# jzlianglu/pykaldi2

Hardware: AMD Instinct MI355X
Metric: iRTF (hrs audio/hr) 3x512 BLSTM LF-MMI, LibriSpeech-shaped synthetic utterances (higher is better)
Workload: dtype f32 (GEMMs: bf16x3 split, f32 accumulate)

## Files before the change

include/pk2hip.h:

```cpp
#ifndef PK2HIP_H_
#define PK2HIP_H_

#include <stddef.h>
#include <stdint.h>

#ifdef __cplusplus
extern "C" {
#endif

typedef enum {
  PK2_OK = 0,
  PK2_ERR_INVALID = -1,
  PK2_ERR_HIP = -2,
  PK2_ERR_LIMIT = -3,
  PK2_ERR_IO = -4,
  PK2_ERR_NUMERIC = -5
} pk2_status;

const char* pk2_last_error(void);
int pk2_version(void);

typedef struct pk2_den_graph pk2_den_graph;

int pk2_den_graph_create(int32_t num_states, int32_t num_pdfs, int64_t num_arcs,
// ... 212 lines not shown
                                int64_t ignore_index, int64_t rows, int32_t num_classes,
                                float* loss_sum, int32_t* count, float* grad, int64_t grad_row_stride, void* stream);
int pk2_scale_inplace_ratio(float* data, int64_t n, const float* num_dev, const float* den_dev, void* stream);
int pk2_scale_by_count(float* data, int64_t n, float numerator, const int32_t* count_den,
                       void* stream);
int pk2_scale_by_scalars(const float* in, float* out, int64_t n, const float* mul_dev, const int32_t* count_den_dev,
                         void* stream);

int pk2_gemm_f32(int32_t transa, int32_t transb, int32_t M, int32_t N, int32_t K, float alpha,
                 const float* A, int64_t lda, const float* B, int64_t ldb, float beta, float* C,
                 int64_t ldc, const float* bias, void* stream);
int pk2_gemm_f32_act(int32_t transa, int32_t transb, int32_t M, int32_t N, int32_t K, float alpha,
                     const float* A, int64_t lda, const float* B, int64_t ldb, float beta, float* C,
                     int64_t ldc, const float* bias, int32_t act, const float* gate, int64_t ldg, void* stream);
int pk2_gemm_f32_seg(int32_t transa, int32_t transb, int32_t M, int32_t N, int32_t K, int32_t nseg, float alpha,
                     const float* A, int64_t lda, int64_t segA, const float* B, int64_t ldb, int64_t segB, float beta,
                     float* C, int64_t ldc, const float* bias, int32_t act, const float* gate, int64_t ldg,
                     void* stream);
int pk2_gemm_f32_batched(int32_t transa, int32_t transb, int32_t M, int32_t N, int32_t K, float alpha,
                         const float* A, int64_t lda, int64_t strideA0, int64_t strideA1, const float* B,
                         int64_t ldb, int64_t strideB0, int64_t strideB1, float beta, float* C, int64_t ldc,
                         int64_t strideC0, int64_t strideC1, int32_t n0, int32_t n1, void* stream);
int pk2_gemm_set_arith(int32_t arith);
int pk2_gemm_get_arith(void);
int pk2_gemm_f32_tn_colsum(int32_t M, int32_t N, int32_t K, float alpha, const float* A, int64_t lda, const float* B,
                           int64_t ldb, float beta, float* C, int64_t ldc, float* colsum, void* stream);
int pk2_colsum_f32(const float* A, int64_t lda, int32_t M, int32_t N, float beta, float* out,
                   void* stream);

size_t pk2_lstm_fwd_workspace_floats(int32_t B, int32_t H, int32_t num_dirs);
int pk2_lstm_layer_fwd(const float* gx, const float* whh, const float* bhh, int32_t B, int32_t T,
                       int32_t H, int32_t num_dirs, float* y, float* gates, float* cells,
                       void* workspace, void* stream);
int pk2_lstm_persist_status(uint32_t* abort_flag);
#define PK2_LSTM_PATH_NONE 0
#define PK2_LSTM_PATH_SEQ 1
#define PK2_LSTM_PATH_BIG 2
#define PK2_LSTM_PATH_BIG_AG 3
#define PK2_LSTM_PATH_STEP_SMALL 4
#define PK2_LSTM_PATH_STEP_BIG 5
int pk2_lstm_last_path(int32_t* fwd, int32_t* bwd);
size_t pk2_lstm_bwd_scratch_floats(int32_t B, int32_t H, int32_t num_dirs);
int pk2_lstm_layer_bwd(const float* dy, const float* whh, const float* gates, const float* cells,
                       int32_t B, int32_t T, int32_t H, int32_t num_dirs, float* dgx,
                       float* scratch, void* stream);
int pk2_lstm_layer_bwd_bias(const float* dy, const float* whh, const float* gates, const float* cells,
                            int32_t B, int32_t T, int32_t H, int32_t num_dirs, float* dgx, float* scratch,
                            float* dbias_ih, float* dbias_hh, int32_t* bias_done, void* stream);
size_t pk2_lstm_bwd_wgrad_workspace_floats(int32_t B, int32_t H, int32_t num_dirs);
int pk2_lstm_layer_bwd_wgrad(const float* dy, const float* whh, const float* gates, const float* cells, const float* y,
                             int32_t B, int32_t T, int32_t H, int32_t num_dirs, float* dgx, float* scratch,
                             float* dbias_ih, float* dbias_hh, float* dwhh, float* wgrad_ws, int32_t* bias_done,
                             int32_t* whh_done, void* stream);

int pk2_layernorm_fwd(const float* x, const float* res, const float* gamma, const float* beta, int64_t rows,
                      int32_t C, float eps, float* sum_out, float* y, float* mean, float* rstd, void* stream);
int pk2_layernorm_bwd(const float* dy, const float* s, const float* mean, const float* rstd,
                      const float* gamma, int64_t rows, int32_t C, float* ds, float* dgamma, float* dbeta,
                      void* stream);
int pk2_softmax_mask_fwd(float* scores, const float* src_mask, const uint8_t* key_padding, int32_t B, int32_t H,
                         int32_t T, void* stream);
int pk2_softmax_bwd(const float* P, float* dP, int32_t BH, int32_t T, void* stream);

int pk2_attention_fwd(const float* qkv, int32_t T, int32_t B, int32_t H, int32_t head_dim, float scale,
                      const float* src_mask, const uint8_t* key_padding, float dropout_p, uint64_t seed, float* ctx,
                      float* lse, void* stream);
// ... 138 lines not shown
```

pykaldi2_amd/_lib.py:

```python
import ctypes as C
import os

import torch

_HERE = os.path.dirname(os.path.abspath(__file__))
LIB_PATH = os.environ.get("PK2_LIB") or os.path.join(_HERE, "libpk2hip.so")


class Pk2Error(RuntimeError):
    pass


class NumBatch(C.Structure):
    _fields_ = [("arc_src", C.c_void_p), ("arc_dst", C.c_void_p), ("arc_pdf", C.c_void_p),
                ("arc_weight", C.c_void_p), ("frame_off", C.c_void_p), ("state_off", C.c_void_p),
                ("final_state", C.c_void_p), ("final_weight", C.c_void_p), ("final_off", C.c_void_p),
                ("total_arcs", C.c_int64), ("max_seq_arcs", C.c_int64)]


class DecoderOpts(C.Structure):
    _fields_ = [("beam", C.c_float), ("lattice_beam", C.c_float), ("beam_delta", C.c_float),
                ("acoustic_scale", C.c_float), ("max_active", C.c_int32), ("min_active", C.c_int32),
                ("tokens_per_frame", C.c_int32), ("links_per_frame", C.c_int32)]

# ... 137 lines not shown
    "pk2_pad_roll_subsample": (C.c_int, [_vp, _vp, _i32, _i32, _i32, _i32, _vp, _i32, _i32, _vp]),
    "pk2_mvn_apply": (C.c_int, [_vp, _vp, _vp, _i64, _i32, _vp, _vp]),
    "pk2_softmax_ce_fwd_bwd": (C.c_int, [_vp, _i64, _vp, _i64, _i64, _i32, _vp, _vp, _vp, _i64, _vp, _vp]),
    "pk2_softmax_ce_fwd_bwd_mean": (C.c_int, [_vp, _i64, _vp, _i64, _i64, _i32, _vp, _vp, _vp, _i64, _vp]),
    "pk2_scale_inplace_ratio": (C.c_int, [_vp, _i64, _vp, _vp, _vp]),
    "pk2_scale_by_count": (C.c_int, [_vp, _i64, _f32, _vp, _vp]),
    "pk2_scale_by_scalars": (C.c_int, [_vp, _vp, _i64, _vp, _vp, _vp]),
    "pk2_gemm_f32": (C.c_int, [_i32, _i32, _i32, _i32, _i32, _f32, _vp, _i64, _vp, _i64, _f32, _vp, _i64,
                               _vp, _vp]),
    "pk2_gemm_f32_act": (C.c_int, [_i32, _i32, _i32, _i32, _i32, _f32, _vp, _i64, _vp, _i64, _f32, _vp, _i64, _vp, _i32, _vp, _i64,
                                   _vp]),
    "pk2_gemm_f32_seg": (C.c_int, [_i32, _i32, _i32, _i32, _i32, _i32, _f32, _vp, _i64, _i64, _vp, _i64, _i64, _f32, _vp, _i64, _vp,
                                   _i32, _vp, _i64, _vp]),
    "pk2_gemm_f32_batched": (C.c_int, [_i32, _i32, _i32, _i32, _i32, _f32, _vp, _i64, _i64, _i64, _vp, _i64, _i64, _i64,
                                       _f32, _vp, _i64, _i64, _i64, _i32, _i32, _vp]),
    "pk2_gemm_f32_tn_colsum": (C.c_int, [_i32, _i32, _i32, _f32, _vp, _i64, _vp, _i64, _f32, _vp, _i64, _vp, _vp]),
    "pk2_gemm_set_arith": (C.c_int, [_i32]),
    "pk2_gemm_get_arith": (C.c_int, []),
    "pk2_layernorm_fwd": (C.c_int, [_vp, _vp, _vp, _vp, _i64, _i32, _f32, _vp, _vp, _vp, _vp, _vp]),
    "pk2_layernorm_bwd": (C.c_int, [_vp, _vp, _vp, _vp, _vp, _i64, _i32, _vp, _vp, _vp, _vp]),
    "pk2_softmax_mask_fwd": (C.c_int, [_vp, _vp, _vp, _i32, _i32, _i32, _vp]),
    "pk2_softmax_bwd": (C.c_int, [_vp, _vp, _i32, _i32, _vp]),
    "pk2_attention_fwd": (C.c_int, [_vp, _i32, _i32, _i32, _i32, _f32, _vp, _vp, _f32, C.c_uint64, _vp, _vp, _vp]),
    "pk2_attention_bwd": (C.c_int, [_vp, _vp, _vp, _vp, _i32, _i32, _i32, _i32, _f32, _vp, _vp, _f32, C.c_uint64, _vp,
                                    _vp, _vp]),
    "pk2_attention_bwd_part": (C.c_int, [_i32, _vp, _vp, _vp, _vp, _i32, _i32, _i32, _i32, _f32, _vp, _vp, _f32, C.c_uint64,
                                         _vp, _vp, _vp]),
    "pk2_relu_fwd": (C.c_int, [_vp, _i64, _vp]),
    "pk2_relu_bwd": (C.c_int, [_vp, _vp, _i64, _vp]),
    "pk2_add_inplace": (C.c_int, [_vp, _vp, _i64, _vp]),
    "pk2_colsum_f32": (C.c_int, [_vp, _i64, _i32, _i32, _f32, _vp, _vp]),
    "pk2_lstm_fwd_workspace_floats": (_sz, [_i32, _i32, _i32]),
    "pk2_lstm_layer_fwd": (C.c_int, [_vp, _vp, _vp, _i32, _i32, _i32, _i32, _vp, _vp, _vp, _vp, _vp]),
    "pk2_lstm_persist_status": (C.c_int, [C.POINTER(C.c_uint32)]),
    "pk2_lstm_last_path": (C.c_int, [C.POINTER(_i32), C.POINTER(_i32)]),
    "pk2_lattice_determinize": (C.c_int, [_i32, _i32, _i64, _vp, _vp, _vp, _vp, _vp, _vp, _vp, C.c_double, _i64, C.POINTER(_vp)]),
    "pk2_det_lattice_sizes": (C.c_int, [_vp, C.POINTER(_i32), C.POINTER(_i32), C.POINTER(_i64), C.POINTER(_i64), C.POINTER(_i64)]),
    "pk2_det_lattice_export": (C.c_int, [_vp] * 12),
    "pk2_det_lattice_destroy": (None, [_vp]),
    "pk2_persist_guard_status": (C.c_int, [C.POINTER(C.c_uint32)]),
    "pk2_persist_guard_clear": (C.c_int, []),
    "pk2_persist_guard_raise": (C.c_int, [_vp]),
    "pk2_persist_guard_export": (C.c_int, [_vp, _vp]),
    "pk2_persist_guard_import": (C.c_int, [_vp, C.c_uint32, _vp]),
    "pk2_persist_guard_verdict": (C.c_int, [C.c_uint32, C.POINTER(C.c_uint32), C.POINTER(C.c_uint32)]),
    "pk2_lstm_bwd_scratch_floats": (_sz, [_i32, _i32, _i32]),
    "pk2_lstm_layer_bwd_bias": (C.c_int, [_vp, _vp, _vp, _vp, _i32, _i32, _i32, _i32, _vp, _vp, _vp, _vp, C.POINTER(_i32), _vp]),
    "pk2_lstm_layer_bwd": (C.c_int, [_vp, _vp, _vp, _vp, _i32, _i32, _i32, _i32, _vp, _vp, _vp]),
    "pk2_lstm_bwd_wgrad_workspace_floats": (_sz, [_i32, _i32, _i32]),
    "pk2_lstm_layer_bwd_wgrad": (C.c_int, [_vp, _vp, _vp, _vp, _vp, _i32, _i32, _i32, _i32, _vp, _vp, _vp, _vp, _vp, _vp,
                                           C.POINTER(_i32), C.POINTER(_i32), _vp]),
    "pk2_dropout_f32": (C.c_int, [_vp, _vp, _i64, _f32, C.c_uint64, _vp]),
    "pk2_grad_norm": (C.c_int, [_vp, _i64, _vp, _vp, _sz, _vp]),
    "pk2_grad_norm_workspace_bytes": (_sz, [_i64]),
    "pk2_adam_step": (C.c_int, [_vp, _vp, _vp, _vp, _vp, _i64, _f32, _f32, _f32, _f32, _f32, _i64, _f32,
                                _vp, _f32, _vp]),
    "pk2_sgd_step": (C.c_int, [_vp, _vp, _vp, _i64, _f32, _f32, _f32, _i32, _f32, _vp, _f32, _vp]),
    "pk2_stream_create_cu_mask": (C.c_int, [_i32, C.POINTER(_vp)]),
    "pk2_stream_destroy": (C.c_int, [_vp]),
    "pk2_debug_where": (C.c_int, [_vp, _i32, _vp]),
    "pk2_debug_peer_reduce": (C.c_int, [_vp, _vp, _i64, _i32, _i32, _vp]),
}

_lib = None


# ... 61 lines not shown
```

pykaldi2_amd/csrc/lstm.hip:

```cpp
#include <algorithm>

#include "common.h"
#include "gemm_tile.h"
#include "lstm_persist.h"
#include "step_graph.h"

namespace pk2 {

typedef float f32x4 __attribute__((ext_vector_type(4)));

constexpr int kFwdThreads = 256;
constexpr int kFwdUnits = 4;

__device__ __forceinline__ float fast_sigmoid(float x) {
  return __builtin_amdgcn_rcpf(1.0f + __builtin_amdgcn_exp2f(-1.4426950408889634f * x));
}
__device__ __forceinline__ float fast_tanh(float x) {
  return 1.0f - 2.0f * __builtin_amdgcn_rcpf(1.0f + __builtin_amdgcn_exp2f(2.8853900817779268f * x));
}

struct LstmFwdParams {
  const float* gx;
  const float* whh;
  const float* bhh;
// ... 434 lines not shown
    const LstmFwdParams* pbb = slot->params;
    const StepCounter* cb = slot->counter;
    char keyb[64];
    snprintf(keyb, sizeof(keyb), "lstm_fwd_big_H%d_D%d_Z%d_%p", H, D, (int)gridb.z, (void*)stream);
    rc = g_graphs.run(keyb, T, slot->counter, stream, [&](hipStream_t s, int j) {
      hipLaunchKernelGGL(lstm_fwd_step_big, gridb, dim3(256), 0, s, pbb, cb, j);
    });
    if (rc) return rc;
    PK2_LAUNCH_CHECK();
    g_last_fwd_path = PK2_LSTM_PATH_STEP_BIG;
    return PK2_OK;
  }
  const int zf = ((B + 15) / 16 + kFwdTileGroup - 1) / kFwdTileGroup;
  dim3 grid(H / kFwdUnits, D, zf), block(kFwdThreads);
  const LstmFwdParams* pb = slot->params;
  const StepCounter* c = slot->counter;
  char key[64];
  snprintf(key, sizeof(key), "lstm_fwd_H%d_D%d_Z%d_%p", H, D, zf, (void*)stream);
  rc = g_graphs.run(key, T, slot->counter, stream, [&](hipStream_t s, int j) {
    switch (H) {
      case 64: launch_step(lstm_fwd_step<4>, grid, block, s, pb, c, j); break;
      case 128: launch_step(lstm_fwd_step<8>, grid, block, s, pb, c, j); break;
      case 256: launch_step(lstm_fwd_step<16>, grid, block, s, pb, c, j); break;
      case 512: launch_step(lstm_fwd_step<32>, grid, block, s, pb, c, j); break;
      default: launch_step(lstm_fwd_step<64>, grid, block, s, pb, c, j); break;
    }
  });
  if (rc) return rc;
#ifdef PK2_LSTM_PROFILE
  hipLaunchKernelGGL(lstm_prof_print, dim3(1), dim3(1), 0, stream, T - 1);
#endif
  PK2_LAUNCH_CHECK();
  g_last_fwd_path = PK2_LSTM_PATH_STEP_SMALL;
  return PK2_OK;
}

extern "C" int pk2_lstm_persist_status(uint32_t* abort_flag) {
  PK2_REQUIRE(abort_flag, "lstm_persist_status: null pointer");
  PK2_HIP(hipDeviceSynchronize());
  unsigned f = 0, f2 = 0;
  int rc = lstm_seq_status(&f);
  if (!rc) rc = lstm_big_status(&f2);
  *abort_flag = f | f2;
  return rc;
}

extern "C" size_t pk2_lstm_bwd_scratch_floats(int32_t B, int32_t H, int32_t D) {
  return (size_t)D * H * 4 * H + (size_t)D * B * H + 64 + (B >= kBigBatch ? (size_t)kBigSplitK * D * B * H : 0);
}

static int lstm_layer_bwd_impl(const float* dy, const float* whh, const float* gates, const float* cells, int32_t B, int32_t T,
                               int32_t H, int32_t D, float* dgx, float* scratch, float* dbias_ih, float* dbias_hh,
                               int32_t* bias_done, void* stream_, SeqWgradCall* wgrad = nullptr);

extern "C" int pk2_lstm_layer_bwd(const float* dy, const float* whh, const float* gates, const float* cells,
                                  int32_t B, int32_t T, int32_t H, int32_t D, float* dgx, float* scratch,
                                  void* stream_) {
  return lstm_layer_bwd_impl(dy, whh, gates, cells, B, T, H, D, dgx, scratch, nullptr, nullptr, nullptr, stream_);
}

extern "C" int pk2_lstm_layer_bwd_bias(const float* dy, const float* whh, const float* gates, const float* cells,
                                       int32_t B, int32_t T, int32_t H, int32_t D, float* dgx, float* scratch,
                                       float* dbias_ih, float* dbias_hh, int32_t* bias_done, void* stream_) {
  PK2_REQUIRE(bias_done, "lstm_bwd_bias: null bias_done");
  return lstm_layer_bwd_impl(dy, whh, gates, cells, B, T, H, D, dgx, scratch, dbias_ih, dbias_hh, bias_done, stream_);
}
// ... 84 lines not shown
```

pykaldi2_amd/csrc/lstm_persist.h:

```cpp
#pragma once
#include "common.h"

namespace pk2 {

bool lstm_seq_wanted(int B, int H, int D);
int lstm_fwd_seq_launch(const float* gx, const float* whh, const float* bhh, int B, int T, int H, int D, float* y,
                        float* gates, float* cells, hipStream_t stream, bool* ran);
struct SeqWgradCall { const float* y; float* dwhh; float* ws; bool done; };
size_t lstm_seq_wgrad_workspace_floats(int B, int H, int D);
int lstm_bwd_seq_launch(const float* dy, const float* whh, const float* gates, const float* cells, int B, int T, int H,
                        int D, float* dgx, hipStream_t stream, bool* ran, float* dbias_ih = nullptr, float* dbias_hh = nullptr,
                        bool* bias_done = nullptr, SeqWgradCall* wgrad = nullptr);
int lstm_seq_status(unsigned* abort_flag);

bool lstm_big_wanted(int B, int H, int D);
int lstm_fwd_big_launch(const float* gx, const float* whh, const float* bhh, int B, int T, int H, int D, float* y,
                        float* gates, float* cells, hipStream_t stream, bool* ran);
int lstm_bwd_big_launch(const float* dy, const float* whh, const float* gates, const float* cells, int B, int T, int H,
                        int D, float* dgx, hipStream_t stream, bool* ran, bool* all_gather);
int lstm_big_status(unsigned* abort_flag);

}
```

pykaldi2_amd/csrc/lstm_persist_seq.hip:

```cpp
#include <algorithm>
#include <cstdint>
#include <cstdlib>
#include <map>

#include "common.h"
#include "lstm_persist.h"
#include "persist_guard.h"

namespace pk2 {

typedef float f32x4 __attribute__((ext_vector_type(4)));
typedef unsigned u32x4 __attribute__((ext_vector_type(4)));

constexpr unsigned kSeqSentinel = 0x7fc0dead;
constexpr int kSH = 512;
constexpr int kSWgs = 32;
constexpr int kSeqTeams = 8;
constexpr int kSeqMaxTasks = 64;
constexpr long long kSeqSpinTicks = 1000LL * 1000 * 100;
constexpr int kSeqMailDepth = 8;
constexpr int kSeqMailFloats = kSeqMailDepth * kSWgs * kSWgs * 16;

struct SeqCtl {
  unsigned arrive[8];
// ... 282 lines not shown
#ifdef PK2_SEQ_PROFILE
      asm volatile("" : "+v"(s0), "+v"(s1), "+v"(s2), "+v"(s3));
#endif
      SQ_T(2);
      const float x = pre + (l16 == 0 ? s0 : l16 == 1 ? s1 : l16 == 2 ? s2 : s3);
      const float act = fmaf(act_a, __builtin_amdgcn_rcpf(1.0f + __builtin_amdgcn_exp2f(act_s * x)), act_b);
      const float fg = seq_dpp<0x101>(act), gg = seq_dpp<0x102>(act), og = seq_dpp<0x103>(act);
      cstate = fg * cstate + act * gg;
      const float h = og * seq_tanh(cstate);
      if (unit_lane) seq_store(y_out, h);
      y_out += y_stride;
      SQ_T(3);
      if (gate_lane) outs[buf][out_idx] = act;
      if (unit_lane) outs[buf][64 + uw] = cstate;
      if (w == 2) {
        gxs[(step + 2) % 3][lane] = gnext;
        gnext = *gx_in;
        gx_in += step + 4 < T ? gx_stride : 0;
      }
      if (w == 3 && step > 0) {
        *gates_out = outs[buf ^ 1][lane];
        if (lane < 16) *cells_out = outs[buf ^ 1][64 + lane];
        gates_out += gates_stride; cells_out += cells_stride;
      }
      SQ_T(4);
    }
    __syncthreads();
    if (w == 3) {
      *gates_out = outs[(T - 1) & 1][lane];
      if (lane < 16) *cells_out = outs[(T - 1) & 1][64 + lane];
    }
    SQ_PRINT("lstm_fwd_seq2", "(poll | lds + barrier | product + row sums | gates + h store | lds hand-over, wave 2 / 3 traffic)", T);
    if (tid == 0 && rank == 0) __hip_atomic_fetch_add(&ctl->done, 1u, __ATOMIC_RELAXED, __HIP_MEMORY_SCOPE_AGENT);
    if (!seq_team_barrier(ctl, role, &nbar, s_i)) return;
  }
}

typedef float f32x32 __attribute__((ext_vector_type(32)));
struct SeqNoWgrad {};
__device__ __forceinline__ float (*seq_yring())[kSH] {
  __shared__ __attribute__((aligned(16))) float ring[3][kSH];
  return ring;
}
template <bool WGRAD, typename WG>
__device__ __forceinline__ void lstm_bwd_seq2_body(const SeqBwdParams& p, SeqCtl* ctl, const WG& g) {
  constexpr int H = kSH, G4 = 4 * kSH;
  __shared__ __attribute__((aligned(16))) float dgl[64];
  __shared__ __attribute__((aligned(16))) float cst[3][16][8];
  float (*yring)[kSH] = nullptr;
  if constexpr (WGRAD) yring = seq_yring();
  __shared__ int s_i[8];
  const int tid = threadIdx.x, lane = tid & 63, w = tid >> 6;
  SeqRole role;
  if (!seq_register(ctl, s_i, &role)) return;
  const int rank = role.rank, B = p.B, T = p.T, D = p.D;
  float* mail0 = p.mail + (size_t)role.team_index * kSeqMailFloats;
  const u32x4 sent = {kSeqSentinel, kSeqSentinel, kSeqSentinel, kSeqSentinel};
  const int row = lane >> 4, l16 = lane & 15;
  const bool pw_lane = w == 0 && l16 < 4;
  const int pw_unit = (4 * row + l16) & 15;
  const bool io = w == 1;
  const bool io16 = io && lane < 16;
  unsigned nbar = 0;
  for (int iter = 0; iter <= kSeqMaxTasks; ++iter) {
    const int task = seq_next_task(ctl, role, iter, B * D, s_i);
    if (task < 0) return;
// ... 208 lines not shown
  if (threadIdx.x == 0) { *sticky = 1u; persist_guard_raise(guard_dev, guard_host); }
  for (size_t i = threadIdx.x; i < n; i += blockDim.x) out[i] = __uint_as_float(0x7fc00000u);
}

struct SeqExit { unsigned pairs; int fold; float* out; size_t n; unsigned* sticky; unsigned* guard_dev; unsigned* guard_host; float* mail; size_t mail_n; };
__device__ __forceinline__ void seq_exit_check(SeqCtl* ctl, const SeqExit& x) {
  if (!x.fold) return;
  __shared__ unsigned s_last;
  __syncthreads();
  if (threadIdx.x == 0) s_last = __hip_atomic_fetch_add(&ctl->exited, 1u, __ATOMIC_ACQ_REL, __HIP_MEMORY_SCOPE_AGENT) == gridDim.x - 1u ? 1u : 0u;
  __syncthreads();
  if (!s_last) return;
  const bool good = seq_load_u(&ctl->abort) == 0u && seq_load_u(&ctl->done) == x.pairs && x.fold != 2;
  __syncthreads();
  for (unsigned i = threadIdx.x; i < sizeof(SeqCtl) / sizeof(unsigned); i += blockDim.x) reinterpret_cast<unsigned*>(ctl)[i] = 0u;
  if (good) return;
  if (threadIdx.x == 0) { if (x.fold != 2) *x.sticky = 1u; persist_guard_raise(x.guard_dev, x.guard_host); }
  for (size_t i = threadIdx.x; i < x.n; i += blockDim.x) x.out[i] = __uint_as_float(0x7fc00000u);
  for (size_t i = threadIdx.x; i < x.mail_n; i += blockDim.x) x.mail[i] = __uint_as_float(kSeqSentinel);
}
__global__ void __launch_bounds__(256) lstm_fwd_seq2(SeqFwdParams p, SeqCtl* ctl, SeqExit x) {
  lstm_fwd_seq2_body(p, ctl);
  seq_exit_check(ctl, x);
}
__global__ void __launch_bounds__(256) lstm_bwd_seq2(SeqBwdParams p, SeqCtl* ctl, SeqExit x) {
  lstm_bwd_seq2_body<false>(p, ctl, SeqNoWgrad());
  seq_exit_check(ctl, x);
}
__global__ void __launch_bounds__(256) lstm_bwd_seq2_wgrad(SeqBwdParams p, SeqCtl* ctl, SeqExit x, SeqWgradParams g) {
  lstm_bwd_seq2_body<true>(p, ctl, g);
  seq_exit_check(ctl, x);
}

__global__ void __launch_bounds__(256) lstm_seq_wgrad_reduce(const float* __restrict__ ws, float* __restrict__ dwhh, int B, int D,
                                                             const unsigned* __restrict__ sticky) {
  constexpr size_t kSlice = (size_t)4 * kSH * kSH;
  const size_t i = (size_t)blockIdx.x * 256 + threadIdx.x;
  if (*sticky != 0u) {
    dwhh[i] = __uint_as_float(0x7fc00000u);
    return;
  }
  const float* in = ws + i;
  float sum = in[0];
  for (int b = 1; b < B; ++b) sum += in[(size_t)b * D * kSlice];
  dwhh[i] += sum;
}

struct SeqScratch { SeqCtl* ctl = nullptr; float* mail = nullptr; unsigned* sticky = nullptr; PersistGuard guard;
                    int mail_clean_teams = 0;
                    bool ctl_clean = false; };
static std::map<DevStream, SeqScratch> g_seq_scratch;
static PersistFamily g_seq("lstm_seq");

static void seq_mail_dirty() { for (auto& kv : g_seq_scratch) { kv.second.mail_clean_teams = 0; kv.second.ctl_clean = false; } }

static int seq_scratch(hipStream_t stream, SeqScratch** out) {
  static const bool hooked = (persist_guard_on_clear(seq_mail_dirty), true);
  (void)hooked;
  SeqScratch& sc = g_seq_scratch[dev_stream(stream)];
  if (!sc.ctl) PK2_HIP(hipMalloc(reinterpret_cast<void**>(&sc.ctl), sizeof(SeqCtl)));
  if (!sc.mail) PK2_HIP(hipMalloc(reinterpret_cast<void**>(&sc.mail), (size_t)8 * kSeqTeams * kSeqMailFloats * sizeof(float)));
  if (!sc.sticky) { int rc = g_seq.new_sticky(stream, &sc.sticky); if (rc) return rc; }
  if (!sc.guard.dev) { int rc = persist_guard(&sc.guard); if (rc) return rc; }
  *out = &sc;
  return PK2_OK;
}

static int seq_teams(int pairs) { return std::max(1, std::min(2, (pairs + 7) / 8)); }

bool lstm_seq_wanted(int B, int H, int D) {
  const char* env = getenv("PK2_LSTM_SEQ");
  if (env && atoi(env) == 0) return false;
  if (!g_seq.usable() || H != kSH || B < 1 || B * D > 32 || (D != 1 && D != 2)) return false;
  return device_cu_count() == 8 * kSWgs;
}

int lstm_fwd_seq_launch(const float* gx, const float* whh, const float* bhh, int B, int T, int H, int D, float* y,
                        float* gates, float* cells, hipStream_t stream, bool* ran) {
  *ran = false;
  SeqScratch* sc = nullptr;
  int rc = seq_scratch(stream, &sc);
  if (rc) return rc;
  if (!sc->ctl_clean) PK2_HIP(hipMemsetAsync(sc->ctl, 0, sizeof(SeqCtl), stream));
  sc->ctl_clean = false;
  PK2_HIP(hipMemsetD32Async(reinterpret_cast<hipDeviceptr_t>(y), (int)kSeqSentinel, (size_t)T * B * D * H, stream));
  SeqFwdParams p{gx, whh, bhh, y, gates, cells, B, T, D};
  const bool fold = g_seq.verified();
  const char* tf_e = getenv("PK2_LSTM_SEQ_TEST_FAIL");
  const int fold_mode = fold ? ((tf_e && atoi(tf_e) == 1) ? 2 : 1) : 0;
  const SeqExit ex{(unsigned)(B * D), fold_mode, y, (size_t)T * B * D * H, sc->sticky, sc->guard.dev, sc->guard.host_dev, nullptr, (size_t)0};
  hipLaunchKernelGGL(lstm_fwd_seq2, dim3(8 * kSWgs * seq_teams(B * D)), dim3(256), 0, stream, p, sc->ctl, ex);
  PK2_LAUNCH_CHECK();
  bool ok = false;
  rc = g_seq.verify_first_use(&sc->ctl->abort, &sc->ctl->done, (unsigned)(B * D), stream, &ok);
  if (rc || !ok) return rc;
  if (!fold)
    hipLaunchKernelGGL(lstm_seq_check, dim3(1), dim3(1024), 0, stream, sc->ctl, (unsigned)(B * D), y, (size_t)T * B * D * H, sc->sticky, sc->guard.dev, sc->guard.host_dev);
  sc->ctl_clean = true;
  *ran = true;
  return PK2_OK;
}

static bool seq_wgrad_resident(int teams) {
  static std::map<int, int> fit;
  const int dev = current_device();
  auto it = fit.find(dev);
  if (it == fit.end()) {
    int n = 0;
    if (hipOccupancyMaxActiveBlocksPerMultiprocessor(&n, lstm_bwd_seq2_wgrad, 256, 0) != hipSuccess) { (void)hipGetLastError(); n = 0; }
    it = fit.emplace(dev, n).first;
  }
  return it->second >= teams;
}

static int seq_wgrad_mode() {
  const char* we = getenv("PK2_LSTM_SEQ_WGRAD");
  return we ? atoi(we) : 1;
}
static int seq_wgrad_teams(int pairs) {
  const int mode = seq_wgrad_mode();
  if (mode == 0) return 0;
  if (seq_wgrad_resident(seq_teams(pairs))) return seq_teams(pairs);
  return (mode == 2 && seq_wgrad_resident(1)) ? 1 : 0;
}

size_t lstm_seq_wgrad_workspace_floats(int B, int H, int D) {
  return (lstm_seq_wanted(B, H, D) && seq_wgrad_teams(B * D) > 0) ? (size_t)B * D * 4 * H * H : 0;
}

int lstm_bwd_seq_launch(const float* dy, const float* whh, const float* gates, const float* cells, int B, int T, int H,
                        int D, float* dgx, hipStream_t stream, bool* ran, float* dbias_ih, float* dbias_hh, bool* bias_done,
                        SeqWgradCall* wgrad) {
  *ran = false;
// ... 54 lines not shown
```

pykaldi2_amd/lstm.py:

```python
import math
import ctypes
import os

import torch
import torch.nn as nn

from . import _lib


def _gemm(ta, tb, M, N, K, A, lda, B, ldb, C, ldc, bias=None, alpha=1.0, beta=0.0):
    _lib.check(_lib.lib().pk2_gemm_f32(int(ta), int(tb), M, N, K, alpha, A, lda, B, ldb, beta, C, ldc,
                                       bias, _lib.stream_ptr()))


def _p(t, off_floats=0):
    import ctypes
    return ctypes.c_void_p(t.data_ptr() + 4 * off_floats)


class _LSTMParams(nn.Module):

    def __init__(self, input_size, hidden_size, num_layers, bidirectional):
        super().__init__()
        self.input_size, self.hidden_size = input_size, hidden_size
# ... 11 lines not shown
        stdv = 1.0 / math.sqrt(H) if H > 0 else 0
        for w in self.parameters():
            nn.init.uniform_(w, -stdv, stdv)


class _LinearParams(nn.Module):

    def __init__(self, in_features, out_features):
        super().__init__()
        self.weight = nn.Parameter(torch.empty(out_features, in_features))
        self.bias = nn.Parameter(torch.empty(out_features))
        nn.init.kaiming_uniform_(self.weight, a=math.sqrt(5))
        bound = 1 / math.sqrt(in_features) if in_features > 0 else 0
        nn.init.uniform_(self.bias, -bound, bound)


class _LstmAmFunction(torch.autograd.Function):

    @staticmethod
    def forward(ctx, x_tm, model, *params):
        m = model
        T, B, Din = x_tm.shape
        H, D, Lr = m.hidden_size, m.num_dirs, m.num_layers
        dev = x_tm.device
        L = _lib.lib()
        sp = _lib.stream_ptr()
        rows = T * B
        saved = []
        seeds = []
        inp = x_tm.contiguous()
        for l in range(Lr):
            w_ih, w_hh, b_ih, b_hh = m._layer_views(l)
            in_size = inp.shape[-1]
            gx = torch.empty(T, B, D * 4 * H, device=dev, dtype=torch.float32)
            _gemm(0, 1, rows, D * 4 * H, in_size, _p(inp), in_size, _p(w_ih), in_size, _p(gx), D * 4 * H,
                  bias=_p(b_ih))
            y = torch.empty(T, B, D * H, device=dev, dtype=torch.float32)
            gates = torch.empty(D, T, B, 4 * H, device=dev, dtype=torch.float32)
            cells = torch.empty(D, T, B, H, device=dev, dtype=torch.float32)
            nws = L.pk2_lstm_fwd_workspace_floats(B, H, D)
            ws = torch.empty(nws, device=dev, dtype=torch.float32) if nws else None
            _lib.check(L.pk2_lstm_layer_fwd(_p(gx), _p(w_hh), _p(b_hh), B, T, H, D, _p(y), _p(gates), _p(cells),
                                            _p(ws) if ws is not None else None, sp))
            saved.append((inp, y, gates, cells))
            inp = y
            if m.dropout > 0 and m.training and l + 1 < Lr:
                seed = int(torch.empty((), dtype=torch.int64).random_().item()) & 0x7FFFFFFFFFFFFFFF
                seeds.append(seed)
                inp = torch.empty_like(y)
                _lib.check(L.pk2_dropout_f32(_p(y), _p(inp), y.numel(), float(m.dropout), seed, sp))
            else:
                seeds.append(None)
        P = m.output_size
        logits = torch.empty(T, B, P, device=dev, dtype=torch.float32)
        _gemm(0, 1, rows, P, D * H, _p(inp), D * H, _p(m.output_layer.weight), D * H, _p(logits), P,
              bias=_p(m.output_layer.bias))
        ctx.model = m
        ctx.saved = saved
        ctx.seeds = seeds
        ctx.shape = (T, B, Din)
        ctx.need_dx = x_tm.requires_grad
        return logits

    @staticmethod
    def backward(ctx, dlogits):
        m = ctx.model
        T, B, Din = ctx.shape
        H, D, Lr, P = m.hidden_size, m.num_dirs, m.num_layers, m.output_size
        L = _lib.lib()
        sp = _lib.stream_ptr()
        rows = T * B
        dev = dlogits.device
        dlogits = dlogits.contiguous()
        gflat = m._grad_flat()
        gflat.zero_()
        views = m._grad_views(gflat)
# ... 200 lines not shown
```

Before: 4587.

## Fuse LSTM input projection into persistent sequential forward kernel

Adds a variant of the persistent sequential LSTM forward kernel in which four extra waves per workgroup compute the input projection (x·W_ih + b_ih) with MFMA in blocks of 32 timesteps. Results go into an LDS ring that the recurrent waves consume, so the separate gx GEMM and its global-memory round trip are skipped. The path runs only for small B*D, input sizes 80 or 1024, a verified seq path and 16-byte alignment; otherwise Python falls back to the old GEMM plus forward call. The cost is doubled block size, larger LDS use and a sleep-throttled projection pipeline that shares the per-step barrier with the recurrence.

```diff
diff --git a/include/pk2hip.h b/include/pk2hip.h
--- a/include/pk2hip.h
+++ b/include/pk2hip.h
@@ -268,6 +268,10 @@
 int pk2_lstm_layer_fwd(const float* gx, const float* whh, const float* bhh, int32_t B, int32_t T,
                        int32_t H, int32_t num_dirs, float* y, float* gates, float* cells,
                        void* workspace, void* stream);
+int pk2_lstm_layer_fwd_xproj(const float* gx, const float* whh, const float* bhh, int32_t B, int32_t T,
+                             int32_t H, int32_t num_dirs, float* y, float* gates, float* cells, void* workspace,
+                             const float* inp, int32_t in_size, const float* w_ih, const float* b_ih,
+                             int32_t* gx_done, void* stream);
 int pk2_lstm_persist_status(uint32_t* abort_flag);
 #define PK2_LSTM_PATH_NONE 0
 #define PK2_LSTM_PATH_SEQ 1
diff --git a/pykaldi2_amd/_lib.py b/pykaldi2_amd/_lib.py
--- a/pykaldi2_amd/_lib.py
+++ b/pykaldi2_amd/_lib.py
@@ -193,6 +193,8 @@
     "pk2_colsum_f32": (C.c_int, [_vp, _i64, _i32, _i32, _f32, _vp, _vp]),
     "pk2_lstm_fwd_workspace_floats": (_sz, [_i32, _i32, _i32]),
     "pk2_lstm_layer_fwd": (C.c_int, [_vp, _vp, _vp, _i32, _i32, _i32, _i32, _vp, _vp, _vp, _vp, _vp]),
+    "pk2_lstm_layer_fwd_xproj": (C.c_int, [_vp, _vp, _vp, _i32, _i32, _i32, _i32, _vp, _vp, _vp, _vp, _vp, _i32, _vp, _vp,
+                                           C.POINTER(_i32), _vp]),
     "pk2_lstm_persist_status": (C.c_int, [C.POINTER(C.c_uint32)]),
     "pk2_lstm_last_path": (C.c_int, [C.POINTER(_i32), C.POINTER(_i32)]),
     "pk2_lattice_determinize": (C.c_int, [_i32, _i32, _i64, _vp, _vp, _vp, _vp, _vp, _vp, _vp, C.c_double, _i64, C.POINTER(_vp)]),
diff --git a/pykaldi2_amd/csrc/lstm.hip b/pykaldi2_amd/csrc/lstm.hip
--- a/pykaldi2_amd/csrc/lstm.hip
+++ b/pykaldi2_amd/csrc/lstm.hip
@@ -490,6 +490,22 @@
 #endif
   PK2_LAUNCH_CHECK();
   g_last_fwd_path = PK2_LSTM_PATH_STEP_SMALL;
+  return PK2_OK;
+}
+
+extern "C" int pk2_lstm_layer_fwd_xproj(const float* gx, const float* whh, const float* bhh, int32_t B, int32_t T, int32_t H,
+                                        int32_t D, float* y, float* gates, float* cells, void* workspace, const float* inp,
+                                        int32_t in_size, const float* w_ih, const float* b_ih, int32_t* gx_done, void* stream_) {
+  PK2_REQUIRE(gx_done, "lstm_fwd_xproj: null gx_done");
+  *gx_done = 0;
+  PK2_REQUIRE(whh && y && gates && cells && inp && w_ih && B > 0 && T > 0 && in_size > 0 && (D == 1 || D == 2), "lstm_fwd_xproj: bad args");
+  PK2_REQUIRE(lstm_h_ok(H), "lstm_fwd_xproj: hidden size %d unsupported (64,128,256,512,1024)", H);
+  (void)gx; (void)workspace;
+  if (!lstm_seq_wanted(B, H, D)) return PK2_OK;
+  bool ran = false;
+  int prc = lstm_fwd_seq_xproj_launch(inp, in_size, w_ih, b_ih, whh, bhh, B, T, H, D, y, gates, cells, static_cast<hipStream_t>(stream_), &ran);
+  if (prc) return prc;
+  if (ran) { g_last_fwd_path = PK2_LSTM_PATH_SEQ; *gx_done = 1; }
   return PK2_OK;
 }
 
diff --git a/pykaldi2_amd/csrc/lstm_persist.h b/pykaldi2_amd/csrc/lstm_persist.h
--- a/pykaldi2_amd/csrc/lstm_persist.h
+++ b/pykaldi2_amd/csrc/lstm_persist.h
@@ -6,6 +6,8 @@
 bool lstm_seq_wanted(int B, int H, int D);
 int lstm_fwd_seq_launch(const float* gx, const float* whh, const float* bhh, int B, int T, int H, int D, float* y,
                         float* gates, float* cells, hipStream_t stream, bool* ran);
+int lstm_fwd_seq_xproj_launch(const float* inp, int in_size, const float* wih, const float* bih, const float* whh, const float* bhh,
+                              int B, int T, int H, int D, float* y, float* gates, float* cells, hipStream_t stream, bool* ran);
 struct SeqWgradCall { const float* y; float* dwhh; float* ws; bool done; };
 size_t lstm_seq_wgrad_workspace_floats(int B, int H, int D);
 int lstm_bwd_seq_launch(const float* dy, const float* whh, const float* gates, const float* cells, int B, int T, int H,
diff --git a/pykaldi2_amd/csrc/lstm_persist_seq.hip b/pykaldi2_amd/csrc/lstm_persist_seq.hip
--- a/pykaldi2_amd/csrc/lstm_persist_seq.hip
+++ b/pykaldi2_amd/csrc/lstm_persist_seq.hip
@@ -338,6 +338,260 @@
     }
     SQ_PRINT("lstm_fwd_seq2", "(poll | lds + barrier | product + row sums | gates + h store | lds hand-over, wave 2 / 3 traffic)", T);
     if (tid == 0 && rank == 0) __hip_atomic_fetch_add(&ctl->done, 1u, __ATOMIC_RELAXED, __HIP_MEMORY_SCOPE_AGENT);
+    if (!seq_team_barrier(ctl, role, &nbar, s_i)) return;
+  }
+}
+
+struct SeqXprojParams {
+  const float* inp;
+  const float* wih;
+  const float* bih;
+  int K;
+};
+constexpr int kXBlock = 32;
+constexpr int kXPitch = 36;
+#ifndef PK2_SEQ_XSLEEP
+#define PK2_SEQ_XSLEEP 17
+#endif
+constexpr int kXSleep = PK2_SEQ_XSLEEP;
+
+template <int K>
+__device__ __forceinline__ void lstm_fwd_seq2_xproj_body(const SeqFwdParams& p, const SeqXprojParams& xp, SeqCtl* ctl) {
+  constexpr int H = kSH;
+  constexpr int kSlicePitch = 36;
+  constexpr int NCH = (K + 31) / 32;
+  constexpr int NREG = NCH < 16 ? NCH : 16, NLDS = NCH - NREG;
+  static_assert(K % 4 == 0 && NCH >= 1 && NCH <= kXBlock, "a block of 32 iterations holds at most 32 chunks of 16-byte granules");
+  __shared__ __attribute__((aligned(16))) float hs[2][16 * kSlicePitch];
+  __shared__ __attribute__((aligned(16))) float xring[2][kXBlock][64];
+  __shared__ __attribute__((aligned(16))) float xs[2][kXBlock][kXPitch];
+  __shared__ __attribute__((aligned(16))) float wl[NLDS > 0 ? NLDS : 1][2][256][4];
+  __shared__ float outs[2][80];
+  __shared__ int s_i[8];
+  const int tid = threadIdx.x, lane = tid & 63, w = __builtin_amdgcn_readfirstlane(tid >> 6);
+  SeqRole role;
+  if (!seq_register(ctl, s_i, &role)) return;
+  const int rank = role.rank, B = p.B, T = p.T, D = p.D;
+  const int ul = lane >> 4, l16 = lane & 15;
+  const int uw = 4 * (w & 3) + ul;
+  const int gu = 16 * rank + uw;
+  const bool unit_lane = l16 == 0, gate_lane = l16 < 4;
+  const bool poller = w < 2;
+  const int gran = (w & 1) * 64 + lane;
+  const float act_s = l16 == 2 ? -2.8853900817779268f : -1.4426950408889634f;
+  const float act_a = l16 == 2 ? 2.0f : 1.0f, act_b = l16 == 2 ? -1.0f : 0.0f;
+  const int pre_idx = 16 * (l16 & 3) + uw, out_idx = gate_lane ? 16 * l16 + uw : 0;
+  const size_t yrow = (size_t)D * H;
+  unsigned nbar = 0;
+  for (int iter = 0; iter <= kSeqMaxTasks; ++iter) {
+    const int task = seq_next_task(ctl, role, iter, B * D, s_i);
+    if (task < 0) return;
+    const int b = task / D, d = task % D;
+    if (w >= 4) {
+      const int q = tid - 256, pw = w - 4, m = l16, kq = ul;
+      const f32x4 zero4 = {0.f, 0.f, 0.f, 0.f};
+      f32x4 wreg[NREG][2];
+      {
+        const float* wrow = xp.wih + ((size_t)d * 4 * H + (size_t)pw * H + 16 * rank + m) * K;
+        auto wload = [&](int c, int h) -> f32x4 {
+          const int k = 32 * c + 8 * kq + 4 * h;
+          const f32x4 v = *reinterpret_cast<const f32x4*>(wrow + (k < K ? k : 0));
+          return k < K ? v : zero4;
+        };
+#pragma unroll 2
+        for (int c = NREG; c < NCH; ++c) {
+          *reinterpret_cast<f32x4*>(&wl[c - NREG][0][q][0]) = wload(c, 0);
+          *reinterpret_cast<f32x4*>(&wl[c - NREG][1][q][0]) = wload(c, 1);
+        }
+#pragma unroll
+        for (int c = 0; c < NREG; ++c) { wreg[c][0] = wload(c, 0); wreg[c][1] = wload(c, 1); }
+      }
+      f32x4 bi = zero4;
+      if (xp.bih) bi = *reinterpret_cast<const f32x4*>(xp.bih + (size_t)d * 4 * H + (size_t)pw * H + 16 * rank + 4 * kq);
+      const int tq = q >> 3, k4 = q & 7;
+      auto xrow = [&](int block) -> const float* {
+        const int s = min(kXBlock * block + tq, T - 1);
+        const size_t t = d == 0 ? (size_t)s : (size_t)(T - 1 - s);
+        return xp.inp + (t * B + b) * (size_t)K;
+      };
+      auto xload = [&](const float* row, int c) -> f32x4 {
+        const int k = 32 * c + 4 * k4;
+        const f32x4 v = *reinterpret_cast<const f32x4*>(row + (k < K ? k : 0));
+        return k < K ? v : zero4;
+      };
+      const float* xrow_cur = xrow(0);
+      const float* xrow_next = xrow(1);
+      f32x4 xnext = xload(xrow_cur, 0);
+      *reinterpret_cast<f32x4*>(&xs[0][tq][4 * k4]) = xnext;
+      xnext = NCH > 1 ? xload(xrow_cur, 1) : zero4;
+      f32x4 acc0[2] = {zero4, zero4}, acc1[2] = {zero4, zero4};
+      __builtin_amdgcn_s_waitcnt(0x0F70);
+      __syncthreads();
+#ifdef PK2_SEQ_PROFILE
+      long long xq_bar = 0, xq_work = 0;
+#endif
+      const int iters = T + kXBlock;
+      for (int i0 = 0; i0 < iters; i0 += kXBlock) {
+        if (i0 > 0) { xrow_cur = xrow_next; xrow_next = xrow((i0 >> 5) + 1); }
+#pragma unroll
+        for (int c = 0; c < kXBlock; ++c) {
+          const int i = i0 + c;
+          if (i >= iters) break;
+#ifdef PK2_SEQ_PROFILE
+          const long long xq0 = clock64();
+#endif
+          seq_lds_barrier();
+          if (s_i[3]) return;
+#ifdef PK2_SEQ_PROFILE
+          const long long xq1 = clock64();
+          xq_bar += xq1 - xq0;
+#endif
+          if (i0 > 0) __builtin_amdgcn_s_sleep(kXSleep);
+          if ((c + 1) % kXBlock < NCH) *reinterpret_cast<f32x4*>(&xs[(c + 1) & 1][tq][4 * k4]) = xnext;
+          if ((c + 2) % kXBlock < NCH) xnext = xload(c + 2 < kXBlock ? xrow_cur : xrow_next, (c + 2) % kXBlock);
+          if (c < NCH) {
+            f32x4 a0, a1;
+            if (c < NREG) { a0 = wreg[c < NREG ? c : 0][0]; a1 = wreg[c < NREG ? c : 0][1]; }
+            else {
+              a0 = *reinterpret_cast<const f32x4*>(&wl[c < NREG ? 0 : c - NREG][0][q][0]);
+              a1 = *reinterpret_cast<const f32x4*>(&wl[c < NREG ? 0 : c - NREG][1][q][0]);
+            }
+            const float* x0 = &xs[c & 1][m][8 * kq];
+            const float* x1 = &xs[c & 1][16 + m][8 * kq];
+            const f32x4 b00 = *reinterpret_cast<const f32x4*>(x0), b01 = *reinterpret_cast<const f32x4*>(x0 + 4);
+            const f32x4 b10 = *reinterpret_cast<const f32x4*>(x1), b11 = *reinterpret_cast<const f32x4*>(x1 + 4);
+#pragma unroll
+            for (int e = 0; e < 4; ++e) {
+              acc0[e & 1] = __builtin_amdgcn_mfma_f32_16x16x4f32(a0[e], b00[e], acc0[e & 1], 0, 0, 0);
+              acc1[e & 1] = __builtin_amdgcn_mfma_f32_16x16x4f32(a0[e], b10[e], acc1[e & 1], 0, 0, 0);
+            }
+#pragma unroll
+            for (int e = 0; e < 4; ++e) {
+              acc0[e & 1] = __builtin_amdgcn_mfma_f32_16x16x4f32(a1[e], b01[e], acc0[e & 1], 0, 0, 0);
+              acc1[e & 1] = __builtin_amdgcn_mfma_f32_16x16x4f32(a1[e], b11[e], acc1[e & 1], 0, 0, 0);
+            }
+          }
+          if (c == kXBlock - 1) {
+            float (*ring)[64] = xring[(i >> 5) & 1];
+            *reinterpret_cast<f32x4*>(&ring[m][16 * pw + 4 * kq]) = (acc0[0] + acc0[1]) + bi;
+            *reinterpret_cast<f32x4*>(&ring[16 + m][16 * pw + 4 * kq]) = (acc1[0] + acc1[1]) + bi;
+#pragma unroll
+            for (int e = 0; e < 2; ++e) { acc0[e] = zero4; acc1[e] = zero4; }
+          }
+#ifdef PK2_SEQ_PROFILE
+          xq_work += clock64() - xq1;
+#endif
+        }
+      }
+#ifdef PK2_SEQ_PROFILE
+      if (q == 0 && rank == 0 && iter == 0)
+        printf("lstm_fwd_seq2_xproj<%d> projection wave 4, %d iterations: %lld clocks per iteration at the barrier | %lld on its chunk\n", K, iters,
+               xq_bar / iters, xq_work / iters);
+#endif
+      __syncthreads();
+    } else {
+      __builtin_amdgcn_s_setprio(3);
+      f32x2 wa[4][16];
+#pragma unroll
+      for (int g = 0; g < 4; ++g) {
+        const float* wrow = p.whh + ((size_t)d * 4 * H + (size_t)g * H + gu) * H + 32 * l16;
+#pragma unroll
+        for (int i = 0; i < 8; ++i) {
+          const f32x4 v = *reinterpret_cast<const f32x4*>(wrow + i * 4);
+          wa[g][2 * i] = f32x2{v[0], v[1]};
+          wa[g][2 * i + 1] = f32x2{v[2], v[3]};
+        }
+      }
+      const float bias = (gate_lane && p.bhh) ? p.bhh[(size_t)d * 4 * H + (size_t)l16 * H + gu] : 0.f;
+      const ptrdiff_t tdir = d == 0 ? 1 : -1;
+      const size_t t0 = d == 0 ? 0 : (size_t)(T - 1);
+      const ptrdiff_t y_stride = tdir * (ptrdiff_t)((size_t)B * yrow);
+      float* y_out = p.y + (t0 * B + b) * yrow + (size_t)d * H + gu;
+      const float* y_poll = p.y + (t0 * B + b) * yrow + (size_t)d * H + 4 * gran - y_stride;
+      const ptrdiff_t gates_stride = tdir * (ptrdiff_t)((size_t)B * 4 * H), cells_stride = tdir * (ptrdiff_t)((size_t)B * H);
+      float* gates_out = p.gates + (((size_t)d * T + t0) * B + b) * 4 * H + (size_t)(lane >> 4) * H + 16 * rank + (lane & 15);
+      float* cells_out = p.cells + (((size_t)d * T + t0) * B + b) * H + 16 * rank + (lane & 15);
+      __builtin_amdgcn_s_waitcnt(0x0F70);
+      __syncthreads();
+      for (int i = 0; i < kXBlock; ++i) {
+        seq_lds_barrier();
+        if (s_i[3]) return;
+      }
+      float cstate = 0.f;
+      bool timed_out = false;
+      SeqSpin spin(ctl);
+      spin.limit = 10 * kSeqSpinTicks;
+      SQ_T0();
+      for (int step = 0; step < T; ++step) {
+        if (step == 2) { spin.limit = kSeqSpinTicks; spin.t0 = 0; }
+        const int buf = step & 1;
+        if (step > 0 && poller) {
+          u32x4 v = seq_load16(y_poll);
+          while (seq_has_sentinel(v)) {
+            if (spin.expired()) { timed_out = true; break; }
+            v = seq_load16(y_poll);
+          }
+          *reinterpret_cast<u32x4*>(&hs[buf][(gran >> 3) * kSlicePitch + 4 * (gran & 7)]) = v;
+        }
+        y_poll += y_stride;
+        SQ_T(0);
+        if (timed_out) s_i[3] = 1;
+        seq_lds_barrier();
+        SQ_T(1);
+        if (s_i[3]) return;
+        const float pre = xring[(step >> 5) & 1][step & 31][pre_idx] + bias;
+        float s0 = 0.f, s1 = 0.f, s2 = 0.f, s3 = 0.f;
+        if (step > 0) {
+          const float* hq = &hs[buf][l16 * kSlicePitch];
+          f32x2 a0 = {0.f, 0.f}, a1 = a0, a2 = a0, a3 = a0, c0 = a0, c1 = a0, c2 = a0, c3 = a0;
+          f32x4 hva[8];
+#pragma unroll
+          for (int i = 0; i < 8; ++i) hva[i] = *reinterpret_cast<const f32x4*>(hq + 4 * i);
+          __builtin_amdgcn_sched_barrier(0);
+#pragma unroll
+          for (int i = 0; i < 8; ++i) {
+            const f32x4 hv = hva[i];
+            const f32x2 h01 = {hv[0], hv[1]}, h23 = {hv[2], hv[3]};
+            a0 = __builtin_elementwise_fma(wa[0][2 * i], h01, a0); c0 = __builtin_elementwise_fma(wa[0][2 * i + 1], h23, c0);
+            a1 = __builtin_elementwise_fma(wa[1][2 * i], h01, a1); c1 = __builtin_elementwise_fma(wa[1][2 * i + 1], h23, c1);
+            a2 = __builtin_elementwise_fma(wa[2][2 * i], h01, a2); c2 = __builtin_elementwise_fma(wa[2][2 * i + 1], h23, c2);
+            a3 = __builtin_elementwise_fma(wa[3][2 * i], h01, a3); c3 = __builtin_elementwise_fma(wa[3][2 * i + 1], h23, c3);
+          }
+          s0 = (a0[0] + a0[1]) + (c0[0] + c0[1]);
+          s1 = (a1[0] + a1[1]) + (c1[0] + c1[1]);
+          s2 = (a2[0] + a2[1]) + (c2[0] + c2[1]);
+          s3 = (a3[0] + a3[1]) + (c3[0] + c3[1]);
+          seq_row_sum4(s0, s1, s2, s3);
+        }
+#ifdef PK2_SEQ_PROFILE
+        asm volatile("" : "+v"(s0), "+v"(s1), "+v"(s2), "+v"(s3));
+#endif
+        SQ_T(2);
+        const float x = pre + (l16 == 0 ? s0 : l16 == 1 ? s1 : l16 == 2 ? s2 : s3);
+        const float act = fmaf(act_a, __builtin_amdgcn_rcpf(1.0f + __builtin_amdgcn_exp2f(act_s * x)), act_b);
+        const float fg = seq_dpp<0x101>(act), gg = seq_dpp<0x102>(act), og = seq_dpp<0x103>(act);
+        cstate = fg * cstate + act * gg;
+        const float h = og * seq_tanh(cstate);
+        if (unit_lane) seq_store(y_out, h);
+        y_out += y_stride;
+        SQ_T(3);
+        if (gate_lane) outs[buf][out_idx] = act;
+        if (unit_lane) outs[buf][64 + uw] = cstate;
+        if (w == 3 && step > 0) {
+          *gates_out = outs[buf ^ 1][lane];
+          if (lane < 16) *cells_out = outs[buf ^ 1][64 + lane];
+          gates_out += gates_stride; cells_out += cells_stride;
+        }
+        SQ_T(4);
+      }
+      __syncthreads();
+      if (w == 3) {
+        *gates_out = outs[(T - 1) & 1][lane];
+        if (lane < 16) *cells_out = outs[(T - 1) & 1][64 + lane];
+      }
+      SQ_PRINT("lstm_fwd_seq2_xproj", "(poll | lds + barrier | product + row sums | gates + h store | lds hand-over, wave 3 traffic)", T);
+      if (tid == 0 && rank == 0) __hip_atomic_fetch_add(&ctl->done, 1u, __ATOMIC_RELAXED, __HIP_MEMORY_SCOPE_AGENT);
+    }
     if (!seq_team_barrier(ctl, role, &nbar, s_i)) return;
   }
 }
@@ -612,6 +866,12 @@
   seq_exit_check(ctl, x);
 }
 
+template <int K>
+__global__ void __launch_bounds__(512) lstm_fwd_seq2_xproj(SeqFwdParams p, SeqXprojParams xp, SeqCtl* ctl, SeqExit x) {
+  lstm_fwd_seq2_xproj_body<K>(p, xp, ctl);
+  seq_exit_check(ctl, x);
+}
+
 __global__ void __launch_bounds__(256) lstm_seq_wgrad_reduce(const float* __restrict__ ws, float* __restrict__ dwhh, int B, int D,
                                                              const unsigned* __restrict__ sticky) {
   constexpr size_t kSlice = (size_t)4 * kSH * kSH;
@@ -655,21 +915,26 @@
   return device_cu_count() == 8 * kSWgs;
 }
 
-int lstm_fwd_seq_launch(const float* gx, const float* whh, const float* bhh, int B, int T, int H, int D, float* y,
-                        float* gates, float* cells, hipStream_t stream, bool* ran) {
+static int seq_fwd_launch(const SeqFwdParams& p, const SeqXprojParams* xp, int teams, int H, hipStream_t stream, bool* ran) {
   *ran = false;
+  const int B = p.B, T = p.T, D = p.D;
+  float* y = p.y;
   SeqScratch* sc = nullptr;
   int rc = seq_scratch(stream, &sc);
   if (rc) return rc;
   if (!sc->ctl_clean) PK2_HIP(hipMemsetAsync(sc->ctl, 0, sizeof(SeqCtl), stream));
   sc->ctl_clean = false;
   PK2_HIP(hipMemsetD32Async(reinterpret_cast<hipDeviceptr_t>(y), (int)kSeqSentinel, (size_t)T * B * D * H, stream));
-  SeqFwdParams p{gx, whh, bhh, y, gates, cells, B, T, D};
   const bool fold = g_seq.verified();
   const char* tf_e = getenv("PK2_LSTM_SEQ_TEST_FAIL");
   const int fold_mode = fold ? ((tf_e && atoi(tf_e) == 1) ? 2 : 1) : 0;
   const SeqExit ex{(unsigned)(B * D), fold_mode, y, (size_t)T * B * D * H, sc->sticky, sc->guard.dev, sc->guard.host_dev, nullptr, (size_t)0};
-  hipLaunchKernelGGL(lstm_fwd_seq2, dim3(8 * kSWgs * seq_teams(B * D)), dim3(256), 0, stream, p, sc->ctl, ex);
+  if (!xp)
+    hipLaunchKernelGGL(lstm_fwd_seq2, dim3(8 * kSWgs * teams), dim3(256), 0, stream, p, sc->ctl, ex);
+  else if (xp->K == 80)
+    hipLaunchKernelGGL(lstm_fwd_seq2_xproj<80>, dim3(8 * kSWgs * teams), dim3(512), 0, stream, p, *xp, sc->ctl, ex);
+  else
+    hipLaunchKernelGGL(lstm_fwd_seq2_xproj<1024>, dim3(8 * kSWgs * teams), dim3(512), 0, stream, p, *xp, sc->ctl, ex);
   PK2_LAUNCH_CHECK();
   bool ok = false;
   rc = g_seq.verify_first_use(&sc->ctl->abort, &sc->ctl->done, (unsigned)(B * D), stream, &ok);
@@ -679,6 +944,39 @@
   sc->ctl_clean = true;
   *ran = true;
   return PK2_OK;
+}
+
+int lstm_fwd_seq_launch(const float* gx, const float* whh, const float* bhh, int B, int T, int H, int D, float* y,
+                        float* gates, float* cells, hipStream_t stream, bool* ran) {
+  const SeqFwdParams p{gx, whh, bhh, y, gates, cells, B, T, D};
+  return seq_fwd_launch(p, nullptr, seq_teams(B * D), H, stream, ran);
+}
+
+static bool seq_xproj_resident() {
+  static std::map<int, bool> fit;
+  const int dev = current_device();
+  auto it = fit.find(dev);
+  if (it == fit.end()) {
+    int n80 = 0, n1024 = 0;
+    if (hipOccupancyMaxActiveBlocksPerMultiprocessor(&n80, lstm_fwd_seq2_xproj<80>, 512, 0) != hipSuccess) { (void)hipGetLastError(); n80 = 0; }
+    if (hipOccupancyMaxActiveBlocksPerMultiprocessor(&n1024, lstm_fwd_seq2_xproj<1024>, 512, 0) != hipSuccess) { (void)hipGetLastError(); n1024 = 0; }
+    it = fit.emplace(dev, n80 >= 1 && n1024 >= 1).first;
+  }
+  return it->second;
+}
+
+int lstm_fwd_seq_xproj_launch(const float* inp, int in_size, const float* wih, const float* bih, const float* whh, const float* bhh,
+                              int B, int T, int H, int D, float* y, float* gates, float* cells, hipStream_t stream, bool* ran) {
+  *ran = false;
+  const char* xe = getenv("PK2_LSTM_SEQ_XPROJ");
+  const int mode = xe ? atoi(xe) : 1;
+  if (mode == 0 || !g_seq.verified() || (in_size != 80 && in_size != 1024)) return PK2_OK;
+  if (B * D > 8 && mode != 2) return PK2_OK;
+  if ((reinterpret_cast<uintptr_t>(inp) | reinterpret_cast<uintptr_t>(wih) | reinterpret_cast<uintptr_t>(bih)) % 16 != 0) return PK2_OK;
+  if (!seq_xproj_resident()) return PK2_OK;
+  const SeqFwdParams p{nullptr, whh, bhh, y, gates, cells, B, T, D};
+  const SeqXprojParams xp{inp, wih, bih, in_size};
+  return seq_fwd_launch(p, &xp, 1, H, stream, ran);
 }
 
 static bool seq_wgrad_resident(int teams) {
diff --git a/pykaldi2_amd/lstm.py b/pykaldi2_amd/lstm.py
--- a/pykaldi2_amd/lstm.py
+++ b/pykaldi2_amd/lstm.py
@@ -67,16 +67,21 @@
         for l in range(Lr):
             w_ih, w_hh, b_ih, b_hh = m._layer_views(l)
             in_size = inp.shape[-1]
-            gx = torch.empty(T, B, D * 4 * H, device=dev, dtype=torch.float32)
-            _gemm(0, 1, rows, D * 4 * H, in_size, _p(inp), in_size, _p(w_ih), in_size, _p(gx), D * 4 * H,
-                  bias=_p(b_ih))
             y = torch.empty(T, B, D * H, device=dev, dtype=torch.float32)
             gates = torch.empty(D, T, B, 4 * H, device=dev, dtype=torch.float32)
             cells = torch.empty(D, T, B, H, device=dev, dtype=torch.float32)
             nws = L.pk2_lstm_fwd_workspace_floats(B, H, D)
             ws = torch.empty(nws, device=dev, dtype=torch.float32) if nws else None
-            _lib.check(L.pk2_lstm_layer_fwd(_p(gx), _p(w_hh), _p(b_hh), B, T, H, D, _p(y), _p(gates), _p(cells),
-                                            _p(ws) if ws is not None else None, sp))
+            gx_done = ctypes.c_int32(0)
+            _lib.check(L.pk2_lstm_layer_fwd_xproj(None, _p(w_hh), _p(b_hh), B, T, H, D, _p(y), _p(gates), _p(cells),
+                                                  _p(ws) if ws is not None else None, _p(inp), in_size, _p(w_ih), _p(b_ih),
+                                                  ctypes.byref(gx_done), sp))
+            if not gx_done.value:
+                gx = torch.empty(T, B, D * 4 * H, device=dev, dtype=torch.float32)
+                _gemm(0, 1, rows, D * 4 * H, in_size, _p(inp), in_size, _p(w_ih), in_size, _p(gx), D * 4 * H,
+                      bias=_p(b_ih))
+                _lib.check(L.pk2_lstm_layer_fwd(_p(gx), _p(w_hh), _p(b_hh), B, T, H, D, _p(y), _p(gates), _p(cells),
+                                                _p(ws) if ws is not None else None, sp))
             saved.append((inp, y, gates, cells))
             inp = y
             if m.dropout > 0 and m.training and l + 1 < Lr:
```

Measured after the change: 4699, median of 6. +2.4%, better.
